# chu-tianxiang/QuIP-for-all

Measured on AMD Instinct MI355X. Metric: decode tokens/sec bs=1 Llama-7B E8P12 2-bit, 1xMI355X; % HBM roofline, higher is better.
Workload: dtype i8xi8->i32 (fp16 I/O); 1 GPU; Llama-2-7B E8P12 random-init, bs=1 greedy decode, 1 hipGraph replay per token, positions [5, 833) of a 2048-slot static KV cache; layers=32, hidden=4096, ffn=11008, vocab=32000, parallelism=replicas x1 (no collective on the data path)

## Files before the change

quip_for_all_amd/csrc/decode_block.hip:

```cpp
#if defined(QUIP_POLL2) || defined(QUIP_POLL2_STAGGER) || defined(QUIP_ROWS_DIRECT) || defined(QUIP_MLP_PREFETCH) || defined(QUIP_INO_EXACT) || \
    defined(QUIP_QKV_ISSUE_EARLY) || defined(QUIP_OWNER_PREDECODE) || defined(QUIP_ATT_THREADS) || defined(QUIP_OHEAD)
#error "retired A/B switch (QUIP_POLL2, _POLL2_STAGGER, _ROWS_DIRECT, _MLP_PREFETCH, _INO_EXACT, _QKV_ISSUE_EARLY, _OWNER_PREDECODE, _ATT_THREADS, _OHEAD): the alternative was measured and its code removed; DESIGN.md 4.11 (QUIP_OHEAD: 4.13) has the result and the commit that still contains it"
#endif
#include "e8p_gemv_core.hip.h"
#include "attn_query.hip.h"
#include "engine_sync.hip.h"
#include "fht_wg512x.hip.h"
#include "token_tail.hip.h"
#include "block_engine_host.hip.h"

#ifndef QUIP_PREDECODE_DOWN
#define QUIP_PREDECODE_DOWN 2
#endif
#ifndef QUIP_PREDECODE_QKV
#define QUIP_PREDECODE_QKV 2
#endif
#ifndef QUIP_ATT_STAMPS
#define QUIP_ATT_STAMPS 0
#endif
#ifndef QUIP_MLP_STAMPS
#define QUIP_MLP_STAMPS 0
#endif
#if QUIP_MLP_STAMPS
#define MSTAMP(i) BSTAMP((i) < 7 ? 18 + (i) : 21 + (i))
// ... 990 lines not shown
          if (tid < HD) {
            float M = -INFINITY, Lsum = 0.f, o = 0.f;
            for (int q2 = 0; q2 < kParts; ++q2) M = fmaxf(M, s_p[q2 * kPartGran + HD]);
            for (int q2 = 0; q2 < kParts; ++q2) {
              const float mq = s_p[q2 * kPartGran + HD];
              const float ww = mq == -INFINITY ? 0.f : __expf(mq - M);
              Lsum = __builtin_fmaf(s_p[q2 * kPartGran + HD + 1], ww, Lsum);
              o = __builtin_fmaf(s_p[q2 * kPartGran + tid], ww, o);
            }
            s_a[tid] = pos_ok ? (f16)(o / Lsum) : __builtin_bit_cast(f16, (unsigned short)0x7e00);
          }
        }
      } else if (tid < HD) {
        s_a[tid] = pos_ok ? (f16)(pO / pL) : __builtin_bit_cast(f16, (unsigned short)0x7e00);
      }
      ASTAMP(3);
      had::wg_barrier<true>();
      ASTAMP(4);
      if constexpr (kOHead) {
        if (head_wg && tid < 64) {
          const f16x2 av = as_f16x2(*reinterpret_cast<const uint32_t*>(s_a + 2 * tid)), su2 = as_f16x2(suo_raw);
          float y[2] = {had::fmul((float)av.x, (float)su2.x), had::fmul((float)av.y, (float)su2.y)};
          hadw::reg_stage<2, 1>(y);
          hadw::lane_stages<2, 0, 6>(y, tid);
          uint32_t w0, w1;
          esync::pack20x2(y[0], y[1], ebase | (hop + 1u), w0, w1);
          esync::st_granule(zbufs + (size_t)3 * 2048 + hd * 64 + tid, w0, w1);
        }
      } else if (head_wg && tid < 64) {
        const uint32_t pr = *reinterpret_cast<const uint32_t*>(s_a + 2 * tid);
        esync::st_granule(zbufs + (size_t)3 * 2048 + hd * 64 + tid, pr, ebase | (hop + 1u));
      }
      }
      ++hop;
    } else {
      hop += 2;
    }
    BSTAMP(6);
    rederive();
    i32x4 Bo[8];
    uint32_t Bon[kPreW];
    {
      esync::drain();
      own_slots(SLOTS(M_O));
      WSTAMP(2);
      if constexpr (NIB) decode_pre(3, Bon);
      else if constexpr (!RVQ) decode_item(3, Bo);
      if constexpr (kOHead) {
        const int jq = 4 * wave + (lane & 3), hp = lane >> 2;
        const uint32_t t16 = (ebase | hop) & 0xffffu;
        {
          uint32_t sp = 0;
          u32x2_t f;
          const uint64_t* g1 = zbufs + (size_t)3 * 2048 + (size_t)((8 * w + wave) & (NH - 1)) * 64;
          for (;;) {
            esync::ld8(f, g1);
            esync::drain();
            esync::own(f);
            if (esync::spin_step((f.y >> 16) == t16, sp, ctl + 1, 0x6100u + (uint32_t)w)) break;
          }
        }
        u32x4_t p[2];
        {
          uint32_t spins = 0;
          const uint64_t* src = zbufs + (size_t)3 * 2048 + (size_t)(2 * hp) * 64 + 2 * jq;
          for (;;) {
            esync::ld16(p[0], src);
            esync::ld16(p[1], src + 64);
            esync::drain();
            esync::own(p[0]);
            esync::own(p[1]);
            const bool ok = (p[0].y >> 16) == t16 && (p[0].w >> 16) == t16 && (p[1].y >> 16) == t16 && (p[1].w >> 16) == t16;
            if (esync::spin_step(ok, spins, ctl + 1, 0x6000u + (uint32_t)w)) break;
          }
        }
        if constexpr (G8) ISSUE8_GU(Ld, 0); else ISSUE(Ld, 4);
        BSTAMP(7);
        float v[8];
#pragma unroll
        for (int r = 0; r < 2; ++r) {
          esync::unpack20x2(p[r].x, p[r].y, v[4 * r], v[4 * r + 1]);
          esync::unpack20x2(p[r].z, p[r].w, v[4 * r + 2], v[4 * r + 3]);
        }
        {
#pragma clang fp contract(off)
          float n0 = 0.f;
#pragma unroll
          for (int r = 0; r < 8; ++r) n0 = __builtin_fmaf(v[r], v[r], n0);
          n0 = had::wave_reduce_to_lane63<false>(n0);
          if (lane == 63) red[wave] = n0;
        }
        hadw::reg_stages<8, 4>(v);
        hadw::lane_stages<8, 2, 6>(v, lane);
        if constexpr (G8) ISSUE8_GU(Ld, 1); else ISSUE(Ld, 5);
        const float sco = Ld.sc[3];
        had::wg_barrier<true>();
        const int sh = norm_shift(red_sum8(0) * (1.f / 128.f), sco);
        if constexpr (G8) ISSUE8_GU(Ld, 2); else ISSUE(Ld, 6);
        {
#pragma clang fp contract(off)
          const float s2 = had::fmul(sco, as_f32((uint32_t)(sh + 127) << 23));
          constexpr int kPS = NIB ? B::PSH : 4096;
#pragma unroll
          for (int r = 0; r < 2; ++r) {
            const float vv[4] = {v[4 * r], v[4 * r + 1], v[4 * r + 2], v[4 * r + 3]};
            uint32_t dh, dm, dl;
            hadw::digit_words_magic(vv, s2, dh, dm, dl);
            const int kd = 32 * (2 * hp + r) + jq;
            const uint32_t off = NIB ? (uint32_t)((kd & 1) * B::HOH + 4 * (kd >> 1)) : (uint32_t)(4 * kd);
            *reinterpret_cast<uint32_t*>(smem + B::kArea + off) = dh;
            *reinterpret_cast<uint32_t*>(smem + B::kArea + kPS + off) = dm;
            *reinterpret_cast<uint32_t*>(smem + B::kArea + 2 * kPS + off) = dl;
          }
        }
        if (tid == 0) shs[3] = sh;
        had::wg_barrier<true>();
      } else {
        u32x4 psu = *reinterpret_cast<const u32x4*>(Ld.su[3] + 8 * tid);
        float v[1][8];
        {
          uint32_t sp = 0;
          u32x2_t f;
          const uint64_t* g1 = zbufs + (size_t)3 * 2048 + (size_t)((8 * w + wave) & (NH - 1)) * 64;
          for (;;) {
            esync::ld8(f, g1);
            esync::drain();
            esync::own(f);
            if (esync::spin_step(f.y == (ebase | hop), sp, ctl + 1, 0x6100u + (uint32_t)w)) break;
          }
        }
        gather(std::integral_constant<int, 1>{}, SLOTS(RVQ ? M_O : 0u), 3, ebase | hop, 0x6000u, v);
        asm volatile("" : "+v"(psu));
        if constexpr (RVQ) ISSUE_RVQ_GATE_G(Ld, 0); else if constexpr (G8) ISSUE8_GU(Ld, 0); else ISSUE(Ld, 4);
        BSTAMP(7);
        had::mul8(v[0], make_uint4(psu.x, psu.y, psu.z, psu.w));
        {
#pragma clang fp contract(off)
          float n0 = 0.f;
#pragma unroll
          for (int r = 0; r < 8; ++r) n0 = __builtin_fmaf(v[0][r], v[0][r], n0);
          n0 = had::wave_reduce_to_lane63<false>(n0);
          if ((tid & 63) == 63) red[wave] = n0;
        }
        had8::fht4096<1, true>(v, xbuf, tid);
        if constexpr (RVQ) ISSUE_RVQ_GATE_G(Ld, 1); else if constexpr (G8) ISSUE8_GU(Ld, 1); else ISSUE(Ld, 5);
        const float sco = Ld.sc[3];
        had::wg_barrier<true>();
        const int sh = norm_shift(red_sum8(0), sco);
        if constexpr (RVQ) ISSUE_RVQ_GATE_G(Ld, 2); else if constexpr (G8) ISSUE8_GU(Ld, 2); else ISSUE(Ld, 6);
        if constexpr (HI) had8::planes_scatter_hi(v[0], sco, sh, reinterpret_cast<uint8_t*>(smem + B::kArea), tid);
        else if constexpr (RVQ) had8::planes_scatter_rvq(v[0], sco, a.resid_scale, sh, reinterpret_cast<uint8_t*>(smem + B::kArea), tid);
        else if constexpr (NIB) {
#pragma clang fp contract(off)
          const float s2 = had::fmul(sco, as_f32((uint32_t)(sh + 127) << 23));
          uint8_t* pb = reinterpret_cast<uint8_t*>(smem + B::kArea) + nib_half_of(tid) * B::HOH + nib_byte_of(tid);
#pragma unroll
          for (int k = 0; k < 8; ++k) {
            const int X = (int)__builtin_rintf(v[0][k] * s2);
            const int X1 = (X + 128) >> 8;
            const int H = (X1 + 128) >> 8;
            uint8_t* p = pb + 256 * k;
            p[0] = (uint8_t)H;
            p[B::PSH] = (uint8_t)X1;
            p[2 * B::PSH] = (uint8_t)X;
          }
        }
        else had8::planes_scatter(v[0], sco, sh, reinterpret_cast<uint8_t*>(smem + B::kArea), tid);
        if (tid == 0) shs[3] = sh;
        had::wg_barrier<true>();
      }
    }
    BSTAMP(8);
    if constexpr (RVQ) {
      run_item(6, xlane, 48);
      run_item(7, xlane + 4096u, 48);
    } else {
      if constexpr (NIB) { Frag Fo; frags(xlane, Fo); add_rows(mul_pre(Bon, Fo), 48); }
      else add_rows(item_multiply(Bo, xlane), 48);
    }
    had::wg_barrier<true>();
    ++hop;
    publish16(4, w * 8, 48, shs[3], ebase | hop);
    had::wg_barrier<true>();
    zero_acc(48, 16);
    BSTAMP(9);

    rederive();
#if QUIP_PREDECODE_GATE
    uint32_t Bg[kPreG][kPreW];
    if constexpr (!RVQ) {
      esync::drain();
      own_slots(SLOTS(M_GATE));
#pragma unroll
      for (int i = 0; i < kPreG; ++i) decode_pre(i, Bg[i]);
    }
#endif
    constexpr int HPIECES = B::kHadElems / 8, NHP = (HPIECES + kThreads - 1) / kThreads, OPIECES = RPO * 3 * (FL / 8);
    static_assert(OPIECES <= kThreads, "one piece of the owner vectors per thread");
    u32x4 fim[NHP], ovec = {0u, 0u, 0u, 0u};
#pragma unroll
    for (int i = 0; i < NHP; ++i) {
      const int pi = tid + kThreads * i;
      fim[i] = reinterpret_cast<const u32x4*>(Ld.had3)[pi < HPIECES ? pi : tid];
    }
    if (w < NRO) {
      const int p = tid < OPIECES ? tid : 0;
      const int row = p / (3 * (FL / 8)), rem = p - row * (3 * (FL / 8));
      const int vsel = rem / (FL / 8), piece = rem - vsel * (FL / 8);
      const int kr = RPO * w + row < FK ? RPO * w + row : FK - 1;
      ovec = *reinterpret_cast<const u32x4*>((vsel == 0 ? Ld.sv[4] : (vsel == 1 ? Ld.sv[5] : Ld.su[6])) + (size_t)kr * FL + piece * 8);
    }
    auto land_mlp_vectors = [&]() {
#pragma unroll
      for (int i = 0; i < NHP; ++i) {
        asm volatile("" : "+v"(fim[i]));
        if (tid + kThreads * i < HPIECES) *reinterpret_cast<u32x4*>(smem + B::kHad + (tid + kThreads * i) * 16) = fim[i];
      }
      asm volatile("" : "+v"(ovec));
      if (w < NRO && tid < OPIECES) *reinterpret_cast<u32x4*>(smem + B::kStash + tid * 16) = ovec;
    };
    edge(std::true_type{}, std::integral_constant<int, 2>{}, SLOTS(M_GATE), 4, ebase | hop, 0x7000u, Ld.sv[3], Ld.ln[1], Ld.su[4 + mgu], Ld.su[4 + mgu], Ld.sc[4 + mgu], Ld.sc[4 + mgu], false,
         [&]() { land_mlp_vectors(); BSTAMP(10); if constexpr (RVQ) ISSUE_RVQ_UP_A_G(Ld, 0); else if constexpr (G8) { ISSUE8_GU(Ld, 3); ISSUE8_GU(Ld, 4); } else ISSUE(Ld, 7); },
         [&]() { if constexpr (RVQ) ISSUE_RVQ_UP_A_G(Ld, 1); else if constexpr (G8) ISSUE8_GU(Ld, 5); else ISSUE(Ld, 8); },
         [&]() { if constexpr (RVQ) ISSUE_RVQ_UP_A_G(Ld, 2); else if constexpr (G8) ISSUE8_GU(Ld, 6); else ISSUE(Ld, 9); }, 18);
    BSTAMP(11);
    MSTAMP(0);
    if constexpr (RVQ || G8) {
      esync::drain();
      own_slots(SLOTS(M_GATE | M_UP));
    }
    MSTAMP(1);
    static_assert(FRB == 3, "three row blocks per matrix");
    if constexpr (RVQ) {
      const uint32_t xu = xlane;
      run_items3(0, xlane, xlane, xlane, 64);
      ISSUE_RVQ_UP_B(Ld);
      run_items3(3, xlane + 4096u, xlane + 4096u, xlane + 4096u, 64);
      run_items3(6, xu, xu, xu, 64 + 16 * FRB);
      esync::drain();
      own_slots(SLOTS(0x007u));
      run_items3(0, xu + 4096u, xu + 4096u, xu + 4096u, 64 + 16 * FRB);
    } else {
      if constexpr (G8) {
        Frag A;
        frags(xlane, A);
#if QUIP_PREDECODE_GATE
#define PRE_G(i) ((i) < kPreG ? Bg[(i) < kPreG ? (i) : 0] : nullptr)
#else
#define PRE_G(i) nullptr
#endif
        add_rows(item_vs(std::integral_constant<int, 0>{}, PRE_G(0), A), B::AGU);
        add_rows(item_vs(std::integral_constant<int, 1>{}, PRE_G(1), A), B::AGU + 16);
        MSTAMP(2);
        add_rows(item_vs(std::integral_constant<int, 2>{}, nullptr, A), B::AGU + 32);
        add_rows(item_vs(std::integral_constant<int, 3>{}, nullptr, A), B::AGU + 48);
        ISSUE8_DOWN(Ld, 0); ISSUE8_DOWN(Ld, 1); ISSUE8_DOWN(Ld, 2); ISSUE8_DOWN(Ld, 3);
        add_rows(item_vs(std::integral_constant<int, 4>{}, nullptr, A), B::AGU + 64);
        add_rows(item_vs(std::integral_constant<int, 5>{}, nullptr, A), B::AGU + 80);
        add_rows(item_vs(std::integral_constant<int, 6>{}, nullptr, A), B::AGU + 96);
#undef PRE_G
      } else {
        Frag A;
        frags(xlane, A);
        auto first_col = [&](auto ic) {
          constexpr int I = decltype(ic)::value;
#if QUIP_PREDECODE_GATE
          if constexpr (I < kPreG) { add_rows(mul_pre(Bg[I < kPreG ? I : 0], A), 64 + 16 * I); return; }
#endif
          add_rows(mul_slot(qa[I], qb[I], A), 64 + 16 * I);
        };
        auto live = [&](auto slot_c, auto behind_c) {
          constexpr int S = decltype(slot_c)::value;
          esync::wait_all_but<decltype(behind_c)::value>();
          own_slots(SLOTS(1u << S));
          add_rows(mul_slot(qa[S], qb[S], A), 64 + 16 * S);
        };
        first_col(std::integral_constant<int, 0>{});
        ISSUE(Ld, 10);
        first_col(std::integral_constant<int, 1>{});
        ISSUE(Ld, 11);
        first_col(std::integral_constant<int, 2>{});
        MSTAMP(2);
        ISSUE(Ld, 12);
        WSTAMP(3);
        live(std::integral_constant<int, 3>{}, std::integral_constant<int, 4 + 6>{});
        WSTAMP(4);
        live(std::integral_constant<int, 4>{}, std::integral_constant<int, 2 + 6>{});
        live(std::integral_constant<int, 5>{}, std::integral_constant<int, 6>{});
        WSTAMP(5);
      }
    }
    WSTAMP(6);
    MSTAMP(3);
    had::wg_barrier<true>();
    BSTAMP(12);

    rederive();
    {
      float* zcol = reinterpret_cast<float*>(smem + B::kZcol);
      if (tid < 16 * NGU) {
        const int m = G8 ? (tid >= FK ? 1 : 0) : tid / 48, k = G8 ? tid - FK * m : tid - 48 * m;
        const int* s3 = accs + (B::AGU + tid) * 4;
        const float f = __builtin_fmaf((float)s3[0], 65536.f, __builtin_fmaf((float)s3[1], 256.f, (float)s3[2]));
        zcol[m * B::KP16 + k] = (float)(f16)(f * unscale_of(shs[0], kUnsc));
      }
      had::wg_barrier<true>();
      zero_acc(B::AGU, 16 * NGU);
      ++hop;
      const uint32_t tag1 = ebase | hop;
      {
        const int o = tid >> 2, part = tid & 3;
        const int m = o >> 6, kq = o & 63;
        const bool live = kq < FK;
        const f16* hs = reinterpret_cast<const f16*>(smem + B::kHad) + mgu * B::KKP + (live ? kq : 0) * FK;
        const float* zz = zcol + m * B::KP16;
        float t = 0.f;
#pragma unroll
        for (int k4 = 0; k4 < (FK + 3) / 4; ++k4) {
          const int k = 4 * k4 + part;
          if (k < FK) t = __builtin_fmaf((float)hs[k], zz[k], t);
        }
        t += __shfl_xor(t, 1, 64);
        t += __shfl_xor(t, 2, 64);
        t *= kMixScale;
        const float tn = __shfl_down(t, 4, 64);
        if (live && part == 0 && (kq & 1) == 0) {
          uint64_t* dst = inbox + (((size_t)(kq / RPO) * FL + (2 * (w & 127) + m)) * (2 * RPO) + mgu * RPO + (kq % RPO));
          if (kq + 1 < FK) esync::st_granule2(dst, as_u32(t), as_u32(tn), tag1);
          else esync::st_granule(dst, as_u32(t), tag1);
        }
      }
      ++hop;
      const uint32_t tag2 = ebase | hop;
      BSTAMP(13);
#if QUIP_PREDECODE_DOWN
      uint32_t Bd[kPreD][kPreW];
      if constexpr (!RVQ) {
        esync::drain();
        own_slots(SLOTS(M_DOWN));
#pragma unroll
        for (int i = 0; i < kPreD; ++i) decode_pre(SDf(i), Bd[i]);
      }
#endif
      if (w < NRO) {
        {
          constexpr int NPC = FL * RPO / kThreads;
          u32x4_t pc[NPC];
          uint32_t spins = 0;
          for (;;) {
#pragma unroll
            for (int jj = 0; jj < NPC; ++jj) esync::ld16(pc[jj], inbox + ((size_t)w * FL * 2 * RPO + 2 * (tid + kThreads * jj)));
            esync::drain();
            bool ok = true;
#pragma unroll
            for (int jj = 0; jj < NPC; ++jj) {
              esync::own(pc[jj]);
              const int kl = 2 * ((tid + kThreads * jj) % (RPO / 2));
              ok = ok && (RPO * w + kl >= FK || pc[jj].y == tag1) && (RPO * w + kl + 1 >= FK || pc[jj].w == tag1);
            }
            if (esync::spin_step(ok, spins, ctl + 1, 0x1000u + (uint32_t)w)) break;
          }
          if (dbg_on && tid == 0) a.dbg[w * 32 + 25] = __builtin_amdgcn_s_memtime();
          uint32_t* rowbuf = reinterpret_cast<uint32_t*>(smem + B::kArea);
#pragma unroll
          for (int jj = 0; jj < NPC; ++jj) {
            const int pi = tid + kThreads * jj, col = pi / RPO, mm = (pi / (RPO / 2)) & 1, kl = 2 * (pi % (RPO / 2));
            rowbuf[(kl * 2 + mm) * FL + col] = pc[jj].x;
            rowbuf[((kl + 1) * 2 + mm) * FL + col] = pc[jj].z;
          }
          had::wg_barrier<true>();
          MSTAMP(4);
        }
        const int rw = wave & (RPO - 1), mh = (wave / RPO) & 1;
        const bool act = wave < 2 * RPO;
        const bool row_ok = RPO * w + rw < FK;
        auto fht256 = [&](float (&x)[4]) {
#pragma clang fp contract(off)
          const float a0 = x[0] + x[1], a1 = x[0] - x[1], a2 = x[2] + x[3], a3 = x[2] - x[3];
          x[0] = a0 + a2; x[2] = a0 - a2; x[1] = a1 + a3; x[3] = a1 - a3;
          auto lst = [&](auto sc) {
            constexpr int S = decltype(sc)::value;
            const float sg = ((lane >> S) & 1) ? -1.f : 1.f;
#pragma unroll
            for (int r = 0; r < 4; ++r) x[r] = __builtin_fmaf(x[r], sg, had8::lane_partner<S>(x[r], lane));
          };
          lst(std::integral_constant<int, 0>{}); lst(std::integral_constant<int, 1>{}); lst(std::integral_constant<int, 2>{});
          lst(std::integral_constant<int, 3>{}); lst(std::integral_constant<int, 4>{}); lst(std::integral_constant<int, 5>{});
        };
        float v[4] = {0.f, 0.f, 0.f, 0.f};
        const f16* vecs = reinterpret_cast<const f16*>(smem + B::kStash) + (row_ok ? rw : 0) * 3 * FL;
        float o[4] = {0.f, 0.f, 0.f, 0.f};
        if (act) {
          {
            const float4 f0 = *reinterpret_cast<const float4*>(reinterpret_cast<const float*>(smem + B::kArea) +
                                                              ((row_ok ? rw : 0) * 2 + mh) * FL + lane * 4);
            v[0] = f0.x; v[1] = f0.y; v[2] = f0.z; v[3] = f0.w;
          }
          fht256(v);
          const uint2 svp = *reinterpret_cast<const uint2*>(vecs + mh * FL + lane * 4);
          const f16x2 s01 = as_f16x2(svp.x), s23 = as_f16x2(svp.y);
          const float svf[4] = {(float)s01.x, (float)s01.y, (float)s23.x, (float)s23.y};
#pragma unroll
          for (int r = 0; r < 4; ++r) o[r] = (float)had::out_elem(v[r], 1.f / 16.f, true, svf[r], false, 0.f, false, 0.f);
        }
        float* xch = reinterpret_cast<float*>(smem + B::kStage + RPO * FL * 4);
        if (act && mh == 1) *reinterpret_cast<float4*>(xch + rw * FL + lane * 4) = float4{o[0], o[1], o[2], o[3]};
        MSTAMP(5);
        had::wg_barrier<true>();
        MSTAMP(6);
        uint32_t* stage = reinterpret_cast<uint32_t*>(smem + B::kStage);
        if (act && mh == 0) {
          const float4 u4 = *reinterpret_cast<const float4*>(xch + rw * FL + lane * 4);
          const float u[4] = {u4.x, u4.y, u4.z, u4.w};
          const uint2 sup = *reinterpret_cast<const uint2*>(vecs + 2 * FL + lane * 4);
          const f16x2 s01 = as_f16x2(sup.x), s23 = as_f16x2(sup.y);
          const float suf[4] = {(float)s01.x, (float)s01.y, (float)s23.x, (float)s23.y};
          float e[4];
#pragma unroll
          for (int r = 0; r < 4; ++r) e[r] = had::fmul(had::fmul(u[r], had::silu(o[r])), suf[r]);
          fht256(e);
          constexpr float kPre = 1.f / 16.f;
          uint16_t* stage16 = reinterpret_cast<uint16_t*>(stage);
#pragma unroll
          for (int r = 0; r < 4; ++r)
            stage16[(4 * lane + r) * RPO + rw] = __builtin_bit_cast(uint16_t, (f16)(e[r] * kPre));
        }
        MSTAMP(7);
        had::wg_barrier<true>();
        if (tid < FL / 2) {
          static_assert(RPO == 2, "one fp16 pair per column and owner");
          const uint2 d = *reinterpret_cast<const uint2*>(stage + 2 * tid);
          esync::st_granule2(frow + ((size_t)w * FL + 2 * tid), d.x, d.y, tag2);
        }
      }
      BSTAMP(14);
      typedef _Float16 f16x4 __attribute__((ext_vector_type(4)));
      constexpr int KCT = B::KP16 / 16;
      u32x2_t arow[2][KCT];
      {
        static_assert(NRO % 2 == 0 && NRO > 8 * (KCT - 1) && NRO <= 8 * KCT, "only q groups of the last k step are beyond the owners");
        if (wave == 0) {
          uint32_t spins0 = 0;
          const uint64_t* last = frow + ((size_t)(lane < NRO ? lane : 0) * FL + (FL - 1 - (w & 7)));
          for (;;) {
            u32x2_t f;
            esync::ld8(f, last);
            esync::drain();
            esync::own(f);
            if (esync::spin_step(f.y == tag2, spins0, ctl + 1, 0x3000u + (uint32_t)w)) break;
          }
        }
        had::wg_barrier<true>();
        BSTAMP(26);
        const bool beyond = 8 * (KCT - 1) + 2 * q >= NRO;
        const uint32_t vo_r = (uint32_t)((2 * q * FL + 16 * wave + n) * 8), vo_rl = (uint32_t)(((beyond ? 0 : 2 * q) * FL + 16 * wave + n) * 8);
        u32x2_t g[2][KCT][2];
        uint32_t spins = 0;
        for (;;) {
#pragma unroll
          for (int s = 0; s < KCT; ++s) {
            const char* base = reinterpret_cast<const char*>(frow) + (size_t)s * 8 * FL * 8;
            const uint32_t vo = s == KCT - 1 ? vo_rl : vo_r;
            if (s == 0) esync::ld8_at<0, true>(g[0][s][0], base, vo); else esync::ld8_at<0>(g[0][s][0], base, vo);
            esync::ld8_at<FL * 8>(g[0][s][1], base, vo);
            esync::ld8_at<kWaves * 16 * 8>(g[1][s][0], base, vo);
            esync::ld8_at<kWaves * 16 * 8 + FL * 8>(g[1][s][1], base, vo);
          }
          esync::drain();
          uint32_t diff = 0u;
#pragma unroll
          for (int jt = 0; jt < 2; ++jt)
#pragma unroll
            for (int s = 0; s < KCT; ++s)
#pragma unroll
              for (int hh = 0; hh < 2; ++hh) {
                esync::own(g[jt][s][hh]);
                diff |= (s == KCT - 1 && beyond) ? 0u : (g[jt][s][hh].y ^ tag2);
              }
          if (esync::spin_step(diff == 0u, spins, ctl + 1, 0x2000u + (uint32_t)w)) break;
        }
#pragma unroll
        for (int jt = 0; jt < 2; ++jt)
#pragma unroll
          for (int s = 0; s < KCT; ++s) {
#pragma unroll
            for (int hh = 0; hh < 2; ++hh) {
              const int o = 8 * s + 2 * q + hh;
              const uint32_t msk = (s == KCT - 1 && beyond) ? 0u : ((2 * o + 1 < FK) ? 0xffffffffu : 0x0000ffffu);
              arow[jt][s][hh] = g[jt][s][hh].x & msk;
            }
            esync::own(arow[jt][s]);
          }
        if constexpr (!RVQ) own_slots(SLOTS(M_DOWN));
        BSTAMP(27);
        if constexpr (RVQ) ISSUE_RVQ_DOWN_G0(Ld);
        if constexpr (kPreQkv) {
          if constexpr (G8) { ISSUE8_QKV(Ln, 0); ISSUE8_QKV(Ln, 1); } else { ISSUE(Ln, 0); ISSUE(Ln, 1); }
        }
        float ssr = 0.f;
#pragma unroll
        for (int jt = 0; jt < 2; ++jt)
#pragma unroll
          for (int s = 0; s < KCT; ++s)
#pragma unroll
            for (int hh = 0; hh < 2; ++hh) {
              const f16x2 a0 = as_f16x2(arow[jt][s][hh]);
              ssr = __builtin_fmaf((float)a0.x, (float)a0.x, ssr); ssr = __builtin_fmaf((float)a0.y, (float)a0.y, ssr);
            }
        ssr = had::wave_reduce_to_lane63<false>(ssr);
        if (lane == 63) red[wave] = ssr;
      }
      if constexpr (RVQ) ISSUE_RVQ_DOWN_G1(Ld);
      BSTAMP(15);
      typedef float f32x4 __attribute__((ext_vector_type(4)));
      f32x4 acc[2][KCT];
#pragma unroll
      for (int jt = 0; jt < 2; ++jt)
#pragma unroll
        for (int ct = 0; ct < KCT; ++ct) acc[jt][ct] = f32x4{0.f, 0.f, 0.f, 0.f};
      {
        const f16* hdT = reinterpret_cast<const f16*>(smem + B::kHad) + 2 * B::KKP;
#pragma unroll
        for (int s = 0; s < KCT; ++s) {
          f16x4 bfs[KCT];
#pragma unroll
          for (int ct = 0; ct < KCT; ++ct) bfs[ct] = *reinterpret_cast<const f16x4*>(hdT + (16 * ct + n) * B::KPS + 16 * s + 4 * q);
#pragma unroll
          for (int jt = 0; jt < 2; ++jt) {
            const uint2 apr = make_uint2(arow[jt][s].x, arow[jt][s].y);
            const f16x4 ah = __builtin_bit_cast(f16x4, apr);
#pragma unroll
            for (int ct = 0; ct < KCT; ++ct)
              acc[jt][ct] = __builtin_amdgcn_mfma_f32_16x16x16f16(ah, bfs[ct], acc[jt][ct], 0, 0, 0);
          }
        }
      }
      if constexpr (RVQ) ISSUE_RVQ_DOWN_G2(Ld);
      MSTAMP(8);
      if constexpr (kPreQkv && !G8) ISSUE(Ln, 2);
#if QUIP_WAIT_STAMPS == 2
      if (dbg_on && lane == 0) a.dbg[w * 32 + (wave < 7 ? 18 + wave : 28)] = dbg_rt ? __builtin_amdgcn_s_memrealtime() : __builtin_amdgcn_s_memtime();
#endif
      had::wg_barrier<true>();
#if QUIP_WAIT_STAMPS == 2
      BSTAMP(29);
#endif
      const float in_scale = Ld.sc[6] * 16.f;
      const float bound = sqrtf(red_sum8(0)) * fabsf(in_scale) * (1.0625f / kMixScale);
      const int sh_d = had::shift_for(bound * ((RVQ && !HI) ? fmaxf(1.f, fabsf(a.resid_scale)) : 1.f));
      MSTAMP(9);
      {
        uint8_t* pl = reinterpret_cast<uint8_t*>(smem + B::kArea);
        const float s2 = had::fmul(in_scale, as_f32((uint32_t)(sh_d + 127) << 23));
        const float s2r = had::fmul(had::fmul(in_scale, a.resid_scale), as_f32((uint32_t)(sh_d + 127) << 23));
#pragma unroll
        for (int jt = 0; jt < 2; ++jt) {
          const int tile = wave + jt * kWaves;
#pragma unroll
          for (int ct = 0; ct < KCT; ++ct) {
            const int kc = 16 * ct + n;
            const float av[4] = {acc[jt][ct][0], acc[jt][ct][1], acc[jt][ct][2], acc[jt][ct][3]};
            if (kc < FK) {
              const int kk = kc * FL + 16 * tile + 4 * q;
              if constexpr (HI) {
                const int vv = 2 * (kk & ~7) + (kk & 4);
                const int offa = (vv >> 8) * 272 + (vv & 255), offb = offa + 8;
                const float ea[4] = {av[0], av[2], 0.f, 0.f}, eb[4] = {av[1], av[3], 0.f, 0.f};
                uint32_t h, m, l;
                hadw::digit_words_magic(ea, s2, h, m, l);
                *reinterpret_cast<uint32_t*>(pl + offa) = h;
                *reinterpret_cast<uint32_t*>(pl + B::kPlaneD + offa) = m;
                *reinterpret_cast<uint32_t*>(pl + 2 * B::kPlaneD + offa) = l;
                hadw::digit_words_magic(eb, s2, h, m, l);
                *reinterpret_cast<uint32_t*>(pl + offb) = h;
                *reinterpret_cast<uint32_t*>(pl + B::kPlaneD + offb) = m;
                *reinterpret_cast<uint32_t*>(pl + 2 * B::kPlaneD + offb) = l;
              } else if constexpr (RVQ) {
                const int vv = 2 * (kk & ~7) + (kk & 7);
                const int offr = (vv >> 8) * 272 + (vv & 255), offm = ((vv + 8) >> 8) * 272 + ((vv + 8) & 255);
                uint32_t h, m, l;
                hadw::digit_words_magic(av, s2r, h, m, l);
                *reinterpret_cast<uint32_t*>(pl + offr) = h;
                *reinterpret_cast<uint32_t*>(pl + B::kPlaneD + offr) = m;
                *reinterpret_cast<uint32_t*>(pl + 2 * B::kPlaneD + offr) = l;
                hadw::digit_words_magic(av, s2, h, m, l);
                *reinterpret_cast<uint32_t*>(pl + offm) = h;
                *reinterpret_cast<uint32_t*>(pl + B::kPlaneD + offm) = m;
                *reinterpret_cast<uint32_t*>(pl + 2 * B::kPlaneD + offm) = l;
              } else {
                const int off = NIB ? ((kk >> 2) & 1) * B::HOD + (kk >> 8) * 144 + (((kk & 255) >> 3) << 2) : (kk >> 8) * 272 + (kk & 255);
                uint32_t h, m, l;
                hadw::digit_words_magic(av, s2, h, m, l);
                *reinterpret_cast<uint32_t*>(pl + off) = h;
                *reinterpret_cast<uint32_t*>(pl + B::kPlaneD + off) = m;
                *reinterpret_cast<uint32_t*>(pl + 2 * B::kPlaneD + off) = l;
              }
            }
          }
        }
        for (int i = VM * NFFN + 4 * tid; i < B::KPDV; i += 4 * kThreads) {
          const int off = NIB ? ((i >> 2) & 1) * B::HOD + (i >> 8) * 144 + (((i & 255) >> 3) << 2) : (i >> 8) * 272 + (i & 255);
#pragma unroll
          for (int d = 0; d < 3; ++d) *reinterpret_cast<uint32_t*>(pl + d * B::kPlaneD + off) = 0u;
        }
      }
      MSTAMP(10);
      had::wg_barrier<true>();
      BSTAMP(16);
      esync::drain();
      own_slots(SLOTS(M_DOWN | (kPreQkv ? M_QKV : 0u)));
      WSTAMP(7);
      const uint32_t xlane_d = NIB ? (uint32_t)B::kArea + nib_row_offset(n, B::kPlaneD, B::HOD) + (uint32_t)q * 32u
                                   : (uint32_t)B::kArea + (uint32_t)min(n, 2) * (uint32_t)B::kPlaneD + (uint32_t)q * 64u;
      constexpr uint32_t kSliceD = NIB ? 288u : 544u;
      if constexpr (RVQ) {
#pragma unroll
        for (int i = 0; i < 6; ++i) {
          const int sl = i * kWaves + wave;
          if (sl < B::JDV) {
            ItemAddr ad;
            item_addresses<REP>(qa[i], qb[i], lane_c, lane_c2, ad, lane_c3);
            add_rows(T::kD4 ? item_mfma_d4<272>(ad, xlane_d + (uint32_t)(sl * 544)) : item_mfma<272, R3>(ad, xlane_d + (uint32_t)(sl * 544)), B::AD);
          }
        }
      } else {
#pragma unroll
        for (int i = 0; i < ND; ++i) {
          const int sl = i * kWaves + wave;
          if (sl < JD) {
#if QUIP_PREDECODE_DOWN
            if (i < kPreD) {
              const uint32_t* bs = Bd[i < kPreD ? i : 0];
              if constexpr (NIB) {
                Frag Fd;
                frags_d(xlane_d + (uint32_t)sl * kSliceD, Fd);
                add_rows(mul_pre(bs, Fd), B::AD);
              } else {
                i32x4 Bt[8];
#pragma unroll
                for (int t = 0; t < 8; ++t) Bt[t] = i32x4{(int)bs[4 * t], (int)bs[4 * t + 1], (int)bs[4 * t + 2], (int)bs[4 * t + 3]};
                add_rows(item_multiply<272>(Bt, xlane_d + (uint32_t)(sl * 544)), B::AD);
              }
              continue;
            }
#endif
            if constexpr (NIB) {
              Frag Fd;
              frags_d(xlane_d + (uint32_t)sl * kSliceD, Fd);
              add_rows(mul_slot(qa[SDf(i)], qb[SDf(i)], Fd), B::AD);
            } else {
              ItemAddr ad;
              item_addresses<REP>(qa[SDf(i)], qb[SDf(i)], lane_c, lane_c2, ad, lane_c3);
              add_rows(T::kD4 ? item_mfma_d4<272>(ad, xlane_d + (uint32_t)(sl * 544)) : item_mfma<272, R3>(ad, xlane_d + (uint32_t)(sl * 544)), B::AD);
            }
          }
        }
      }
      WSTAMP(8);
      had::wg_barrier<true>();
      ++hop;
      publish16(5, w * 8, B::AD, sh_d, ebase | hop);
      had::wg_barrier<true>();
      zero_acc(B::AD, 16);
      BSTAMP(17);
    }
    sv_d_prev = Ld.sv[6];
    const bool more = l + 1 < a.n_layers;
    if (more) {
      had::wg_barrier<true>();
      if (tid < 64) reinterpret_cast<uint32_t*>(smem + B::kDesc)[tid] = reinterpret_cast<const uint32_t*>(a.layers + l + 1)[tid];
      had::wg_barrier<true>();
    }
    rederive();
    uint32_t Bq[NPQ][kPreW];
    if constexpr (kPreQkv) {
#pragma unroll
      for (int i = 0; i < NPQ; ++i) decode_pre(SQf(i), Bq[i]);
    }
    {
      const int c_lo = qc_lo, c_hi = qc_hi;
      edge(std::true_type{}, std::integral_constant<int, 2>{}, SLOTS(0u), 5, ebase | hop, 0x4000u, sv_d_prev, Ld.ln[0], Ld.su[c_lo], Ld.su[c_hi],
           Ld.sc[c_lo], Ld.sc[c_hi], c_hi != c_lo,
           [&]() { BSTAMP(1); if constexpr (RVQ) { ISSUE_RVQ_QKV_G(Ld, 0); ISSUE_RVQ_QKV_G(Ld, 1); } else if constexpr (!kPreQkv) { ISSUE(Ld, 0); ISSUE(Ld, 1); } },
           [&]() { if constexpr (RVQ) ISSUE_RVQ_QKV_G(Ld, 2); else if constexpr (!kPreQkv) ISSUE(Ld, 2); }, [&]() {}, 23);
      BSTAMP(2);
    }
    if (more) P1_products(std::integral_constant<bool, kPreQkv>{}, Bq);
    esync::drain();
    own_slots(SLOTS(M_QKV));
  }
  if (whole_token) {
    static_assert(B::kArea % 16 == 0 && B::kAreaBytes >= tail::kLdsBytes, "the tail's x and reduction slots in the transient area");
    const bool tst = a.dbg != nullptr && (a.dbg_layer & 0xffff) == a.n_layers;
    ++hop;
    tail::run(a.tail, hreg, smem + B::kArea, ctl, zbufs, ebase | hop, w, a.rms_eps, pos64, tst ? a.dbg + w * 32 : nullptr, dbg_rt);
  }
  if (w == 0) {
    uint32_t e, fp;
    esync::ld4(e, ctl + 1);
    esync::ld4(fp, ctl + 2);
    esync::drain();
    esync::own(e);
    esync::own(fp);
    const bool failed = __builtin_amdgcn_readfirstlane((int)e) != 0;
    if (a.h_out) {
#pragma unroll
      for (int j = 0; j < 4; ++j) {
        reinterpret_cast<uint16_t*>(a.h_out)[tid + 512 * (2 * j)] = failed ? (uint16_t)0x7e00 : (uint16_t)(hreg[j] & 0xffffu);
        reinterpret_cast<uint16_t*>(a.h_out)[tid + 512 * (2 * j + 1)] = failed ? (uint16_t)0x7e00 : (uint16_t)(hreg[j] >> 16);
      }
    }
    if (tid == 0) {
      if (failed && fp == 0u) esync::st_word(ctl + 2, (uint32_t)pos + 1u);
      esync::st_word(ctl, ebase >> 10);
      if (!failed && (ebase >> 10) >= (1u << 22) - 2u) esync::st_word(ctl + 1, 0xE000u);
    }
  }
#undef BSTAMP
#undef ISSUE
#undef GU_RB
#undef GU_OFF2
#undef GU_COL
// ... 90 lines not shown
```

Measured before the change: 945.3 tokens/s.

## Restructure MLP gate/up mix exchange so one wave per row handles both halves

Changes the z-column shared layout to residue-major so each thread loads its z values as float4 vectors. It also changes the inbox layout so each owner row's gate and up halves are contiguous, and has one wave poll and load its own row directly from global memory. The old path did a block-wide poll, a scatter into shared memory and two barriers. The gate and up Hadamard transforms now run in the same wave (8 values per lane), which removes the LDS exchange and a workgroup barrier. In exchange, half the waves sit idle in this phase, the per-wave register count rises, and the producer and consumer inbox layouts must stay in sync.

```diff
diff --git a/quip_for_all_amd/csrc/decode_block.hip b/quip_for_all_amd/csrc/decode_block.hip
--- a/quip_for_all_amd/csrc/decode_block.hip
+++ b/quip_for_all_amd/csrc/decode_block.hip
@@ -1316,7 +1316,7 @@
         const int m = G8 ? (tid >= FK ? 1 : 0) : tid / 48, k = G8 ? tid - FK * m : tid - 48 * m;
         const int* s3 = accs + (B::AGU + tid) * 4;
         const float f = __builtin_fmaf((float)s3[0], 65536.f, __builtin_fmaf((float)s3[1], 256.f, (float)s3[2]));
-        zcol[m * B::KP16 + k] = (float)(f16)(f * unscale_of(shs[0], kUnsc));
+        zcol[m * B::KP16 + (k & 3) * (B::KP16 / 4) + (k >> 2)] = (float)(f16)(f * unscale_of(shs[0], kUnsc));
       }
       had::wg_barrier<true>();
       zero_acc(B::AGU, 16 * NGU);
@@ -1324,25 +1324,29 @@
       const uint32_t tag1 = ebase | hop;
       {
         const int o = tid >> 2, part = tid & 3;
-        const int m = o >> 6, kq = o & 63;
+        const int m = o & 1, kq = o >> 1;
         const bool live = kq < FK;
         const f16* hs = reinterpret_cast<const f16*>(smem + B::kHad) + mgu * B::KKP + (live ? kq : 0) * FK;
-        const float* zz = zcol + m * B::KP16;
+        constexpr int K4 = (FK + 3) / 4, KQ = B::KP16 / 4;
+        static_assert(B::kZcol % 16 == 0 && KQ % 4 == 0 && K4 <= KQ, "a residue's z values: whole 16-byte pieces");
+        float zz[KQ];
+#pragma unroll
+        for (int i = 0; i < (K4 + 3) / 4; ++i) {
+          const float4 z4 = *reinterpret_cast<const float4*>(zcol + m * B::KP16 + part * KQ + 4 * i);
+          zz[4 * i] = z4.x; zz[4 * i + 1] = z4.y; zz[4 * i + 2] = z4.z; zz[4 * i + 3] = z4.w;
+        }
         float t = 0.f;
 #pragma unroll
-        for (int k4 = 0; k4 < (FK + 3) / 4; ++k4) {
+        for (int k4 = 0; k4 < K4; ++k4) {
           const int k = 4 * k4 + part;
-          if (k < FK) t = __builtin_fmaf((float)hs[k], zz[k], t);
+          if (k < FK) t = __builtin_fmaf((float)hs[k], zz[k4], t);
         }
         t += __shfl_xor(t, 1, 64);
         t += __shfl_xor(t, 2, 64);
         t *= kMixScale;
         const float tn = __shfl_down(t, 4, 64);
-        if (live && part == 0 && (kq & 1) == 0) {
-          uint64_t* dst = inbox + (((size_t)(kq / RPO) * FL + (2 * (w & 127) + m)) * (2 * RPO) + mgu * RPO + (kq % RPO));
-          if (kq + 1 < FK) esync::st_granule2(dst, as_u32(t), as_u32(tn), tag1);
-          else esync::st_granule(dst, as_u32(t), tag1);
-        }
+        if (live && part == 0 && m == 0)
+          esync::st_granule2(inbox + (((size_t)kq * 2 + mgu) * FL + 2 * (w & 127)), as_u32(t), as_u32(tn), tag1);
       }
       ++hop;
       const uint32_t tag2 = ebase | hop;
@@ -1357,81 +1361,66 @@
       }
 #endif
       if (w < NRO) {
-        {
-          constexpr int NPC = FL * RPO / kThreads;
-          u32x4_t pc[NPC];
-          uint32_t spins = 0;
-          for (;;) {
-#pragma unroll
-            for (int jj = 0; jj < NPC; ++jj) esync::ld16(pc[jj], inbox + ((size_t)w * FL * 2 * RPO + 2 * (tid + kThreads * jj)));
-            esync::drain();
-            bool ok = true;
-#pragma unroll
-            for (int jj = 0; jj < NPC; ++jj) {
-              esync::own(pc[jj]);
-              const int kl = 2 * ((tid + kThreads * jj) % (RPO / 2));
-              ok = ok && (RPO * w + kl >= FK || pc[jj].y == tag1) && (RPO * w + kl + 1 >= FK || pc[jj].w == tag1);
+        const int rw = wave & (RPO - 1);
+        const bool act = wave < RPO;
+        const bool row_ok = RPO * w + rw < FK;
+        auto fht256 = [&](auto& x) {
+#pragma clang fp contract(off)
+          constexpr int N = sizeof(x) / sizeof(float);
+#pragma unroll
+          for (int g = 0; g < N; g += 4) {
+            const float a0 = x[g] + x[g + 1], a1 = x[g] - x[g + 1], a2 = x[g + 2] + x[g + 3], a3 = x[g + 2] - x[g + 3];
+            x[g] = a0 + a2; x[g + 2] = a0 - a2; x[g + 1] = a1 + a3; x[g + 3] = a1 - a3;
+          }
+          hadw::lane_stages<N, 0, 6>(x, lane);
+        };
+        const f16* vecs = reinterpret_cast<const f16*>(smem + B::kStash) + (row_ok ? rw : 0) * 3 * FL;
+        uint32_t* stage = reinterpret_cast<uint32_t*>(smem + B::kStage);
+        if (act) {
+          float v[8];
+          {
+            u32x4_t pc[4];
+            const uint64_t* src = inbox + (((size_t)(RPO * w + (row_ok ? rw : 0)) * 2) * FL + 4 * lane);
+            uint32_t spins = 0;
+            for (;;) {
+#pragma unroll
+              for (int j = 0; j < 4; ++j) esync::ld16(pc[j], src + (j >> 1) * FL + 2 * (j & 1));
+              esync::drain();
+              bool ok = true;
+#pragma unroll
+              for (int j = 0; j < 4; ++j) {
+                esync::own(pc[j]);
+                ok = ok && (!row_ok || (pc[j].y == tag1 && pc[j].w == tag1));
+              }
+              if (esync::spin_step(ok, spins, ctl + 1, 0x1000u + (uint32_t)w)) break;
             }
-            if (esync::spin_step(ok, spins, ctl + 1, 0x1000u + (uint32_t)w)) break;
-          }
-          if (dbg_on && tid == 0) a.dbg[w * 32 + 25] = __builtin_amdgcn_s_memtime();
-          uint32_t* rowbuf = reinterpret_cast<uint32_t*>(smem + B::kArea);
-#pragma unroll
-          for (int jj = 0; jj < NPC; ++jj) {
-            const int pi = tid + kThreads * jj, col = pi / RPO, mm = (pi / (RPO / 2)) & 1, kl = 2 * (pi % (RPO / 2));
-            rowbuf[(kl * 2 + mm) * FL + col] = pc[jj].x;
-            rowbuf[((kl + 1) * 2 + mm) * FL + col] = pc[jj].z;
-          }
-          had::wg_barrier<true>();
+            if (dbg_on && tid == 0) a.dbg[w * 32 + 25] = __builtin_amdgcn_s_memtime();
+#pragma unroll
+            for (int j = 0; j < 4; ++j) {
+              v[2 * j] = row_ok ? __builtin_bit_cast(float, (uint32_t)pc[j].x) : 0.f;
+              v[2 * j + 1] = row_ok ? __builtin_bit_cast(float, (uint32_t)pc[j].z) : 0.f;
+            }
+          }
           MSTAMP(4);
-        }
-        const int rw = wave & (RPO - 1), mh = (wave / RPO) & 1;
-        const bool act = wave < 2 * RPO;
-        const bool row_ok = RPO * w + rw < FK;
-        auto fht256 = [&](float (&x)[4]) {
-#pragma clang fp contract(off)
-          const float a0 = x[0] + x[1], a1 = x[0] - x[1], a2 = x[2] + x[3], a3 = x[2] - x[3];
-          x[0] = a0 + a2; x[2] = a0 - a2; x[1] = a1 + a3; x[3] = a1 - a3;
-          auto lst = [&](auto sc) {
-            constexpr int S = decltype(sc)::value;
-            const float sg = ((lane >> S) & 1) ? -1.f : 1.f;
-#pragma unroll
-            for (int r = 0; r < 4; ++r) x[r] = __builtin_fmaf(x[r], sg, had8::lane_partner<S>(x[r], lane));
-          };
-          lst(std::integral_constant<int, 0>{}); lst(std::integral_constant<int, 1>{}); lst(std::integral_constant<int, 2>{});
-          lst(std::integral_constant<int, 3>{}); lst(std::integral_constant<int, 4>{}); lst(std::integral_constant<int, 5>{});
-        };
-        float v[4] = {0.f, 0.f, 0.f, 0.f};
-        const f16* vecs = reinterpret_cast<const f16*>(smem + B::kStash) + (row_ok ? rw : 0) * 3 * FL;
-        float o[4] = {0.f, 0.f, 0.f, 0.f};
-        if (act) {
-          {
-            const float4 f0 = *reinterpret_cast<const float4*>(reinterpret_cast<const float*>(smem + B::kArea) +
-                                                              ((row_ok ? rw : 0) * 2 + mh) * FL + lane * 4);
-            v[0] = f0.x; v[1] = f0.y; v[2] = f0.z; v[3] = f0.w;
-          }
           fht256(v);
-          const uint2 svp = *reinterpret_cast<const uint2*>(vecs + mh * FL + lane * 4);
-          const f16x2 s01 = as_f16x2(svp.x), s23 = as_f16x2(svp.y);
-          const float svf[4] = {(float)s01.x, (float)s01.y, (float)s23.x, (float)s23.y};
-#pragma unroll
-          for (int r = 0; r < 4; ++r) o[r] = (float)had::out_elem(v[r], 1.f / 16.f, true, svf[r], false, 0.f, false, 0.f);
-        }
-        float* xch = reinterpret_cast<float*>(smem + B::kStage + RPO * FL * 4);
-        if (act && mh == 1) *reinterpret_cast<float4*>(xch + rw * FL + lane * 4) = float4{o[0], o[1], o[2], o[3]};
-        MSTAMP(5);
-        had::wg_barrier<true>();
-        MSTAMP(6);
-        uint32_t* stage = reinterpret_cast<uint32_t*>(smem + B::kStage);
-        if (act && mh == 0) {
-          const float4 u4 = *reinterpret_cast<const float4*>(xch + rw * FL + lane * 4);
-          const float u[4] = {u4.x, u4.y, u4.z, u4.w};
+          float svf[8];
+#pragma unroll
+          for (int mh = 0; mh < 2; ++mh) {
+            const uint2 svp = *reinterpret_cast<const uint2*>(vecs + mh * FL + lane * 4);
+            const f16x2 s01 = as_f16x2(svp.x), s23 = as_f16x2(svp.y);
+            svf[4 * mh] = (float)s01.x; svf[4 * mh + 1] = (float)s01.y; svf[4 * mh + 2] = (float)s23.x; svf[4 * mh + 3] = (float)s23.y;
+          }
+          float o[8];
+#pragma unroll
+          for (int r = 0; r < 8; ++r) o[r] = (float)had::out_elem(v[r], 1.f / 16.f, true, svf[r], false, 0.f, false, 0.f);
+          MSTAMP(5);
+          MSTAMP(6);
           const uint2 sup = *reinterpret_cast<const uint2*>(vecs + 2 * FL + lane * 4);
           const f16x2 s01 = as_f16x2(sup.x), s23 = as_f16x2(sup.y);
           const float suf[4] = {(float)s01.x, (float)s01.y, (float)s23.x, (float)s23.y};
           float e[4];
 #pragma unroll
-          for (int r = 0; r < 4; ++r) e[r] = had::fmul(had::fmul(u[r], had::silu(o[r])), suf[r]);
+          for (int r = 0; r < 4; ++r) e[r] = had::fmul(had::fmul(o[4 + r], had::silu(o[r])), suf[r]);
           fht256(e);
           constexpr float kPre = 1.f / 16.f;
           uint16_t* stage16 = reinterpret_cast<uint16_t*>(stage);
```

Measured after the change: 960.6 tokens/s (median of 6 runs). 1.6% higher.
